# FatimaSohailll/KLT-Feature-Tracker-Acceleration-GPUs

Measured on AMD Instinct MI355X. Metric: frames/sec + pyramid Gpix/s @1080p 5000 feats, 1/2/4/8 MI355X, higher is better.
Workload: dtype f32; 1 GPU; 1920x1080, 5000 features, sequential KLTTrackFeatures pass + KLTStoreFeatureList per frame, 2361 frames per GPU (BASELINE config 3; config 5 at N>1); device-resident: frames in HBM before timing, features and table stay on the device (the API-inclusive figure is the `api` key); chunk=64, chunk_requested=64, resolution=1920x1080, features=5000, frames=2361, parallelism=single GPU, reduction=exact

## Files before the change

klt-feature-tracker-acceleration-gpus_amd/csrc/track7.hip:

```cpp
#pragma clang fp contract(off)
#pragma clang diagnostic ignored "-Wpass-failed"

#include <math.h>
#include <string.h>

#include "klt_dev.h"

#ifndef KLT_T7_PRED_UNIT
#define KLT_T7_PRED_UNIT 0
#endif
#ifndef KLT_T7_NL2
#define KLT_T7_NL2 1
#endif
#ifndef KLT_T7_REUSE
#define KLT_T7_REUSE 1
#endif
#ifndef KLT_T7_BATCH
#define KLT_T7_BATCH 7
#endif

namespace kltdev {
namespace {

constexpr int kWin = 7, kHw = 3, kNpx = kWin * kWin;
constexpr int kRow = 52;
constexpr int kRows = 6;
constexpr int kWaves = kBlock / kWave;

__device__ __forceinline__ float u(float v) { return __int_as_float(__builtin_amdgcn_readfirstlane(__float_as_int(v))); }
__device__ __forceinline__ int u(int v) { return __builtin_amdgcn_readfirstlane(v); }

#include "track7_solve.h"

constexpr int kThreeBits = 0x40400000;

__device__ __forceinline__ bool out7(float x, float y, int tx, int ty) {
  const int xb = __float_as_int(x), yb = __float_as_int(y);
  return xb < kThreeBits || xb >= tx || yb < kThreeBits || yb >= ty;
}

struct Pix {
  unsigned off;
  unsigned px;
  float w0, w1, w2, w3;
};

__device__ __forceinline__ Pix pix_at(int w, int h, float x, float y) {
  const int xt = (int)x, yt = (int)y;
  const float ax = x - xt, ay = y - yt;
  Pix p;
  p.px = (unsigned)(yt * w + xt);
  p.off = p.px * 4u;
  p.w0 = (1.0f - ax) * (1.0f - ay);
  p.w1 = ax * (1.0f - ay);
  p.w2 = (1.0f - ax) * ay;
  p.w3 = ax * ay;
  return p;
}

struct Quad {
  float2 r0, r1;
};

__device__ __forceinline__ Quad quad(const float *P, const Pix &p, unsigned rowb) {
  const char *b = reinterpret_cast<const char *>(P);
  const unsigned o1 = p.off + rowb;
  Quad q;
  q.r0 = *reinterpret_cast<const float2 *>(b + p.off);
  q.r1 = *reinterpret_cast<const float2 *>(b + o1);
  return q;
}

typedef float f4u __attribute__((ext_vector_type(4), aligned(4)));
typedef float f2u __attribute__((ext_vector_type(2), aligned(4)));
struct Tri {
  Quad i, x, y;
};
__device__ __forceinline__ Tri tri(const float *P, const Pix &p, unsigned rowb) {
  const char *base = reinterpret_cast<const char *>(P);
  const unsigned o0 = p.px * 12u, o1 = o0 + rowb;
  const f4u a0 = *reinterpret_cast<const f4u *>(base + o0), b0 = *reinterpret_cast<const f4u *>(base + o1);
  const f2u a1 = *reinterpret_cast<const f2u *>(base + o0 + 16), b1 = *reinterpret_cast<const f2u *>(base + o1 + 16);
  static_assert(kRecGx == 0 && kRecGy == 1 && kRecImg == 2, "record layout");
  Tri t;
  t.i.r0 = make_float2(a0.z, a1.y);
  t.i.r1 = make_float2(b0.z, b1.y);
  t.x.r0 = make_float2(a0.x, a0.w);
  t.x.r1 = make_float2(b0.x, b0.w);
  t.y.r0 = make_float2(a0.y, a1.x);
  t.y.r1 = make_float2(b0.y, b1.x);
  return t;
}
__device__ __forceinline__ Quad quad_i(const float *P, const Pix &p, unsigned rowb) {
  const unsigned o0 = p.px * 12u, o1 = o0 + rowb;
  const float *b = reinterpret_cast<const float *>(reinterpret_cast<const char *>(P) + o0);
  const float *c = reinterpret_cast<const float *>(reinterpret_cast<const char *>(P) + o1);
  Quad q;
  q.r0 = make_float2(b[kRecImg], b[kRec + kRecImg]);
  q.r1 = make_float2(c[kRecImg], c[kRec + kRecImg]);
  return q;
}

__device__ __forceinline__ float interp(const Pix &p, const Quad &q) {
  return p.w0 * q.r0.x + p.w1 * q.r0.y + p.w2 * q.r1.x + p.w3 * q.r1.y;
}

#ifndef KLT_T7_WAVEFENCE
#define KLT_T7_WAVEFENCE 1
#endif
__device__ __forceinline__ void wave_lds_sync() {
#if KLT_T7_WAVEFENCE
  __builtin_amdgcn_fence(__ATOMIC_RELEASE, "wavefront");
  __builtin_amdgcn_wave_barrier();
  __builtin_amdgcn_fence(__ATOMIC_ACQUIRE, "wavefront");
#else
  __builtin_amdgcn_fence(__ATOMIC_RELEASE, "workgroup");
  __builtin_amdgcn_wave_barrier();
  __builtin_amdgcn_fence(__ATOMIC_ACQUIRE, "workgroup");
#endif
}

typedef float f4 __attribute__((ext_vector_type(4)));

template <int NS, bool PIN = false>
__device__ __forceinline__ float sums7_acc(float *red, int lane, bool on, const float (&v)[NS]) {
  if (on) {
#pragma unroll
    for (int s = 0; s < NS; ++s) red[s * kRow + lane] = v[s];
  }
  wave_lds_sync();
  float acc = 0.0f;
  if constexpr (PIN) asm volatile("" : "+v"(lane));
  if (lane < NS) {
    const float *r = red + lane * kRow;
    constexpr int NCH = kRow / 4, B = KLT_T7_BATCH;
#pragma unroll
    for (int k0 = 0; k0 < NCH; k0 += B) {
      f4 c[B];
#pragma unroll
      for (int k = 0; k < B; ++k)
        if (k0 + k < NCH) c[k] = *reinterpret_cast<const f4 *>(r + 4 * (k0 + k));
#pragma unroll
      for (int k = 0; k < B; ++k) {
        const int q = 4 * (k0 + k);
        if (k0 + k >= NCH) break;
        acc += c[k].x;
        if (q + 1 < kNpx) acc += c[k].y;
        if (q + 2 < kNpx) acc += c[k].z;
        if (q + 3 < kNpx) acc += c[k].w;
      }
    }
  }
  wave_lds_sync();
  return acc;
}
template <int NS, bool PIN = false>
__device__ __forceinline__ void sums7(float *red, int lane, bool on, const float (&v)[NS], float (&out)[NS]) {
  const float acc = sums7_acc<NS, PIN>(red, lane, on, v);
#pragma unroll
  for (int s = 0; s < NS; ++s) out[s] = __int_as_float(__builtin_amdgcn_readlane(__float_as_int(acc), s));
}

constexpr int kQuadXor1 = 0xB1, kQuadXor2 = 0x4E, kRowRor4 = 0x124, kRowRor8 = 0x128;
constexpr int kRowBcast15 = 0x142, kRowBcast31 = 0x143;
#ifndef KLT_T7_BCAST
#define KLT_T7_BCAST 1
#endif
template <int CTRL>
__device__ __forceinline__ float dpp_add(float x) {
  return x + __int_as_float(__builtin_amdgcn_update_dpp(0, __float_as_int(x), CTRL, 0xF, 0xF, false));
}

template <int NS>
__device__ __forceinline__ void tree7(bool on, const float (&v)[NS], float (&out)[NS]) {
  float x[NS];
#pragma unroll
  for (int s = 0; s < NS; ++s) x[s] = on ? v[s] : 0.0f;
#pragma unroll
  for (int s = 0; s < NS; ++s) x[s] = dpp_add<kQuadXor1>(x[s]);
#pragma unroll
  for (int s = 0; s < NS; ++s) x[s] = dpp_add<kQuadXor2>(x[s]);
#pragma unroll
  for (int s = 0; s < NS; ++s) x[s] = dpp_add<kRowRor4>(x[s]);
#pragma unroll
  for (int s = 0; s < NS; ++s) x[s] = dpp_add<kRowRor8>(x[s]);
#if KLT_T7_BCAST
#pragma unroll
  for (int s = 0; s < NS; ++s) x[s] = x[s] + __int_as_float(__builtin_amdgcn_update_dpp(0, __float_as_int(x[s]),
                                                                                          kRowBcast15, 0xF, 0xF, true));
#pragma unroll
  for (int s = 0; s < NS; ++s) x[s] = x[s] + __int_as_float(__builtin_amdgcn_update_dpp(0, __float_as_int(x[s]),
                                                                                          kRowBcast31, 0xF, 0xF, true));
#pragma unroll
  for (int s = 0; s < NS; ++s) out[s] = __int_as_float(__builtin_amdgcn_readlane(__float_as_int(x[s]), 63));
#else
#pragma unroll
  for (int s = 0; s < NS; ++s) {
    const int b = __float_as_int(x[s]);
    out[s] = (__int_as_float(__builtin_amdgcn_readlane(b, 0)) + __int_as_float(__builtin_amdgcn_readlane(b, 16))) +
             (__int_as_float(__builtin_amdgcn_readlane(b, 32)) + __int_as_float(__builtin_amdgcn_readlane(b, 48)));
  }
#endif
}

template <int NS, bool FAST, bool PIN = false>
__device__ __forceinline__ void sums(float *red, int lane, bool on, const float (&v)[NS], float (&out)[NS]) {
  if constexpr (FAST) tree7<NS>(on, v, out);
  else sums7<NS, PIN>(red, lane, on, v, out);
}

constexpr int kPS = 24;
constexpr int kPatS = 16 * kPS, kPatT = 2 * 16 * 8, kPatG = 2 * 8 * 8;
constexpr int kPat = kPatS + kPatT;
static_assert(kPatG <= kPatS, "G over S");
constexpr int kRedF = kRows * kRow + 4;

typedef float f2 __attribute__((ext_vector_type(2)));

__device__ __forceinline__ void patch_load(const float *img, int w, int h, int X0, int Y0, int lane, float (&v)[4]) {
  const int sc = lane & 15, sr = 2 * ((lane >> 4) & 1) + (lane >> 5);
  const unsigned xc = (unsigned)clampi(X0 - kHw + sc, 0, w - 1);
  const char *b = reinterpret_cast<const char *>(img);
#pragma unroll
  for (int k = 0; k < 4; ++k) {
    const unsigned yc = (unsigned)clampi(Y0 - kHw + sr + 4 * k, 0, h - 1);
    v[k] = *reinterpret_cast<const float *>(b + (yc * (unsigned)w + xc) * 4u);
  }
}

__device__ __forceinline__ void patch_grads(float *pat, int lane, const TrkArgs &a, int w, int h, const float (&v)[4],
                                            int X0, int Y0, int cx, int cy, Quad &qi, Quad &qx, Quad &qy) {
  const int sc = lane & 15, sr = 2 * ((lane >> 4) & 1) + (lane >> 5);
#pragma unroll
  for (int k = 0; k < 4; ++k) pat[(sr + 4 * k) * kPS + sc] = v[k];
  wave_lds_sync();
  {
    const float *S = pat + (cy + kHw) * kPS + cx + kHw;
    qi.r0 = make_float2(S[0], S[1]);
    qi.r1 = make_float2(S[kPS], S[kPS + 1]);
  }
  const int c = lane & 7, r = lane >> 3;
#pragma unroll
  for (int k = 0; k < 2; ++k) {
    const float *row = pat + (r + 8 * k) * kPS + c;
    f2 t = {0.0f, 0.0f};
#pragma unroll
    for (int m = 0; m < 7; ++m) t += f2{row[m], row[m]} * f2{a.gd[m], a.gg[m]};
    float *T = pat + kPatS + 2 * ((r + 8 * k) * 8 + c);
    T[0] = t.y;
    T[1] = t.x;
  }
  wave_lds_sync();
  {
    const float *col = pat + kPatS + 2 * (r * 8 + c);
    f2 g = {0.0f, 0.0f};
#pragma unroll
    for (int m = 0; m < 7; ++m) g += *reinterpret_cast<const f2 *>(col + 16 * m) * f2{a.gd[m], a.gg[m]};
    const int x = X0 + c, y = Y0 + r;
    if (x < kHw || x + kHw >= w || y < kHw || y + kHw >= h) g = f2{0.0f, 0.0f};
    *reinterpret_cast<f2 *>(pat + 2 * (r * 8 + c)) = g;
  }
  wave_lds_sync();
  const int cx1 = min(cx + 1, 7), cy1 = min(cy + 1, 7);
  const f2 g00 = *reinterpret_cast<const f2 *>(pat + 2 * (cy * 8 + cx));
  const f2 g01 = *reinterpret_cast<const f2 *>(pat + 2 * (cy * 8 + cx1));
  const f2 g10 = *reinterpret_cast<const f2 *>(pat + 2 * (cy1 * 8 + cx));
  const f2 g11 = *reinterpret_cast<const f2 *>(pat + 2 * (cy1 * 8 + cx1));
  qx.r0 = make_float2(g00.y, g01.y);
  qx.r1 = make_float2(g10.y, g11.y);
  qy.r0 = make_float2(g00.x, g01.x);
  qy.r1 = make_float2(g10.x, g11.x);
  wave_lds_sync();
}

struct Carry {
  unsigned px = ~0u;
  Quad i, x, y;
};
#ifndef KLT_T7_CARRY
#define KLT_T7_CARRY 1
#endif

struct Lev {
  const float *img, *gx, *gy;
  int w, h, vlo, vhi;
  int tx, ty;
  int il;
};

__device__ __forceinline__ Lev lev_of(const TrkLevel &L, long off, int tx, int ty) {
  return Lev{L.img + off, L.gx + off, L.gy + off, L.w, L.h, L.vlo, L.vhi, tx, ty, L.il};
}

__device__ __forceinline__ Lev lev_prev(const TrkArgs &a, const TrkFramesArgs &b, int r, int j) {
  const TrkLevel &P = a.A[r], &Q = a.B[r];
  const bool f = j == 0;
  const long off = f ? 0L : (long)(j - 1) * b.lfs[r];
  return Lev{(f ? P.img : Q.img) + off, (f ? P.gx : Q.gx) + off, (f ? P.gy : Q.gy) + off, f ? P.w : Q.w,
             f ? P.h : Q.h, f ? P.vlo : Q.vlo, f ? P.vhi : Q.vhi, a.oobx[r], a.ooby[r], f ? P.il : Q.il};
}

template <bool MULTI>
__device__ __forceinline__ Lev lev_cur(const TrkArgs &a, const TrkFramesArgs &b, int r, int j, int sq, int nsq) {
  if constexpr (MULTI) return lev_of(a.B[r], ((long)j * nsq + sq) * b.lfs[r], a.oobx[r], a.ooby[r]);
  else return lev_of(a.B[r], (long)j * b.lfs[r], a.oobx[r], a.ooby[r]);
}
template <bool MULTI>
__device__ __forceinline__ Lev lev_before(const TrkArgs &a, const TrkFramesArgs &b, int r, int j, int sq, int nsq) {
  if constexpr (MULTI) {
    const TrkLevel &P = a.A[r], &Q = a.B[r];
    const bool f = j == 0;
    const long off = (f ? (long)sq : (long)(j - 1) * nsq + sq) * b.lfs[r];
    return Lev{(f ? P.img : Q.img) + off, nullptr, nullptr, Q.w, Q.h, Q.vlo, Q.vhi, a.oobx[r], a.ooby[r], Q.il};
  } else {
    return lev_prev(a, b, r, j);
  }
}

template <bool MULTI, bool ROLL>
__device__ __forceinline__ Lev lev_img1(const TrkArgs &a, const TrkFramesArgs &b, int r, int j, int sq, int nsq,
                                        const float *pimg, int pil) {
  if constexpr (ROLL) {
    const TrkLevel &Q = a.B[r];
    return Lev{pimg, nullptr, nullptr, Q.w, Q.h, Q.vlo, Q.vhi, a.oobx[r], a.ooby[r], pil};
  } else {
    return lev_before<MULTI>(a, b, r, j, sq, nsq);
  }
}

__device__ __forceinline__ bool band_bad(const Lev &L, float y) {
  return (int)(y - kHw) < L.vlo || (int)(y + kHw) + 1 >= L.vhi;
}

struct Pending {
  bool on = false;
  float x2 = 0.0f, y2 = 0.0f;
  int it = 0;
  float aim = 0.0f;
};

struct Counts {
  unsigned solves = 0, passes = 0;
#ifdef KLT_TRACK_PROF
  unsigned long long c[kProfN] = {};
#endif
};

constexpr int kWaveXcdShift = 60;
constexpr unsigned long long kWaveTimeMask = (1ull << kWaveXcdShift) - 1ull;
__device__ __forceinline__ void wave_time(unsigned long long *wave_t, int which, unsigned k) {
  const unsigned long long t = wall_clock64(), cap = wave_t[2];
  const unsigned long long xcd = (unsigned)__builtin_amdgcn_s_getreg((31 << 11) | 20) & 15u;
  if (k < cap) wave_t[4 + which * cap + k] = (t & kWaveTimeMask) | (xcd << kWaveXcdShift);
}
struct T7KArgs {
  TrkArgs a;
  TrkFramesArgs b;
  float *fx, *fy;
  int *fv;
  int n;
};
typedef const __attribute__((address_space(4))) T7KArgs *T7KArgsPtr;
__device__ __forceinline__ T7KArgsPtr t7_kargs() {
  return (T7KArgsPtr)__builtin_amdgcn_kernarg_segment_ptr();
}
__device__ __forceinline__ void wave_exit(int lane, unsigned k) {
  if (lane != 0) return;
  const T7KArgsPtr ka = t7_kargs();
  unsigned long long *const wave_t = ka->b.wave_t;
  unsigned *const exits = ka->b.exits;
  if (wave_t) wave_time(wave_t, 1, k);
  if (exits) {
    const unsigned k = atomicAdd(exits, 1u) + 1u;
    if (k == ka->b.exit_thr) __hip_atomic_store(ka->b.exit_sig, k, __ATOMIC_RELAXED, __HIP_MEMORY_SCOPE_SYSTEM);
  }
}

#ifdef KLT_TRACK_PROF
#define T7_T(t) const unsigned long long t = clock64()
#define T7_ADD(k, t0) cnt.c[k] += clock64() - (t0)
#else
#define T7_T(t)
#define T7_ADD(k, t0)
#endif

struct LevState {
  float x2, y2;
  float pxy;
  float aim, agx, agy;
  int it = 0;
  int status = kTracked;
  unsigned bpx = ~0u;
  Quad bi, bx, by;
};

enum { kPassAgain = 0, kPassDone = 1, kPassOOB = 2, kPassLostPrev = 3 };

template <bool BAND, bool FIRST, bool JOB, bool AOS, bool FAST, int LZ = 0>
__device__ __forceinline__ int pass7(const TrkArgs &a, const Lev &A, const Lev &B, float x1, float y1, bool x1_out,
                                     LevState &ls, int lane, float fi, float fj, bool on, float *red, Pending &pd,
                                     const Lev &R, int &rstat, Counts &cnt, const Carry &cr = Carry{},
                                     unsigned cpx = ~0u) {
  T7_T(t_top);
  if constexpr (KLT_T7_SOLVE2 && !FIRST) ls.x2 = lane_of(ls.pxy, 0), ls.y2 = lane_of(ls.pxy, 1);
  bool stop = (FIRST && x1_out) || out7(ls.x2, ls.y2, A.tx, A.ty);
  if (BAND && !stop && (band_bad(B, ls.y2) || (FIRST && band_bad(A, y1)))) {
    *a.escape = 1;
    stop = true;
  }
  if (stop) {
    ls.status = kOOB;
    if (JOB) {
      const Pix q = pix_at(R.w, R.h, pd.x2 + fi, pd.y2 + fj);
      const float rb =
          interp(q, AOS && !LZ ? quad_i(R.img, q, (unsigned)R.w * 12u) : quad(R.img, q, (unsigned)R.w * 4u));
      float v[1] = {on ? fabsf(pd.aim - rb) : 0.0f}, S[1];
      ++cnt.passes;
      sums<1, FAST, LZ != 0>(red, lane, on, v, S);
      rstat = S[0] / (float)kNpx > a.max_res ? kLargeResidue : (pd.it >= a.max_it ? kMaxIter : kTracked);
      pd.on = false;
      if (rstat != kTracked) return kPassLostPrev;
    }
    return kPassOOB;
  }
  T7_ADD(11, t_top);
  T7_T(t_g0);
  ++cnt.passes;
  const unsigned rowB = (unsigned)B.w * (AOS ? 12u : 4u);
  const Pix qb = pix_at(B.w, B.h, ls.x2 + fi, ls.y2 + fj);
  Quad bi, bx, by;
  const bool reuse = !FIRST && KLT_T7_REUSE && __ballot(qb.px != ls.bpx) == 0ull;
  Pix qa = qb, qr = qb;
  Quad ai{}, ax{}, ay{}, ri{};
  if constexpr (LZ == 2) {
    float *pat = red + kRedF;
    if (FIRST) qa = pix_at(A.w, A.h, x1 + fi, y1 + fj);
    if (JOB) {
      qr = pix_at(R.w, R.h, pd.x2 + fi, pd.y2 + fj);
      ri = quad(R.img, qr, (unsigned)R.w * 4u);
    }
    const int X0b = u((int)(ls.x2 - (float)kHw)), Y0b = u((int)(ls.y2 - (float)kHw));
    const int cxb = (int)(ls.x2 + fi) - X0b, cyb = (int)(ls.y2 + fj) - Y0b;
    const bool carry = FIRST && KLT_T7_CARRY && __ballot(qa.px != cpx) == 0ull;
    if (reuse) {
      bi = ls.bi;
      bx = ls.bx;
      by = ls.by;
    } else if (!FIRST || carry) {
      float v[4];
      patch_load(B.img, B.w, B.h, X0b, Y0b, lane, v);
      patch_grads(pat, lane, a, B.w, B.h, v, X0b, Y0b, cxb, cyb, bi, bx, by);
      if (FIRST) ai = cr.i, ax = cr.x, ay = cr.y;
    } else if (A.il == kLayoutImg) {
      const int X0a = u((int)(x1 - (float)kHw)), Y0a = u((int)(y1 - (float)kHw));
      float v[4], va[4];
      patch_load(B.img, B.w, B.h, X0b, Y0b, lane, v);
      patch_load(A.img, A.w, A.h, X0a, Y0a, lane, va);
      patch_grads(pat, lane, a, B.w, B.h, v, X0b, Y0b, cxb, cyb, bi, bx, by);
      patch_grads(pat, lane, a, A.w, A.h, va, X0a, Y0a, (int)(x1 + fi) - X0a, (int)(y1 + fj) - Y0a, ai, ax, ay);
    } else {
      float v[4];
      patch_load(B.img, B.w, B.h, X0b, Y0b, lane, v);
      const Tri t = tri(A.img, qa, (unsigned)A.w * 12u);
      patch_grads(pat, lane, a, B.w, B.h, v, X0b, Y0b, cxb, cyb, bi, bx, by);
      ai = t.i, ax = t.x, ay = t.y;
    }
  } else if (reuse) {
    bi = ls.bi;
    bx = ls.bx;
    by = ls.by;
  } else if constexpr (AOS) {
    const Tri t = tri(B.img, qb, rowB);
    bi = t.i;
    bx = t.x;
    by = t.y;
  } else {
    bi = quad(B.img, qb, rowB);
    bx = quad(B.gx, qb, rowB);
    by = quad(B.gy, qb, rowB);
  }
  if (KLT_T7_REUSE) {
    ls.bpx = qb.px;
    ls.bi = bi;
    ls.bx = bx;
    ls.by = by;
  }
  if (FIRST && LZ != 2) {
    const unsigned rowA = (unsigned)A.w * (AOS ? 12u : 4u);
    qa = pix_at(A.w, A.h, x1 + fi, y1 + fj);
    if constexpr (AOS) {
      const Tri t = tri(A.img, qa, rowA);
      ai = t.i;
      ax = t.x;
      ay = t.y;
    } else {
      ai = quad(A.img, qa, rowA);
      ax = quad(A.gx, qa, rowA);
      ay = quad(A.gy, qa, rowA);
    }
  }
  if (JOB && LZ != 2) {
    qr = pix_at(R.w, R.h, pd.x2 + fi, pd.y2 + fj);
    ri = AOS && !LZ ? quad_i(R.img, qr, (unsigned)R.w * 12u) : quad(R.img, qr, (unsigned)R.w * 4u);
  }
  if (FIRST) {
    ls.aim = interp(qa, ai);
    ls.agx = interp(qa, ax);
    ls.agy = interp(qa, ay);
  }
  const float bim = interp(qb, bi), bgx = interp(qb, bx), bgy = interp(qb, by);
  const float dif = ls.aim - bim, gxs = ls.agx + bgx, gys = ls.agy + bgy;
#ifdef KLT_TRACK_PROF
  asm volatile("" ::"v"(dif), "v"(gxs), "v"(gys));
#endif
  T7_ADD(0, t_g0);
  T7_T(t_s0);
  constexpr bool S2L = KLT_T7_SOLVE2 && !FAST;
  constexpr int iXX = S2L ? kSumGxx : 0, iXY = S2L ? kSumGxy : 1, iYY = S2L ? kSumGyy : 2, iEX = S2L ? kSumEx : 3,
                iEY = S2L ? kSumEy : 4, iRes = S2L ? kSumRes : 5;
  float S[6], acc = 0.0f;
  if (JOB) {
    const float rb = interp(qr, ri);
    float v[6];
    v[iXX] = gxs * gxs, v[iXY] = gxs * gys, v[iYY] = gys * gys, v[iEX] = dif * gxs, v[iEY] = dif * gys;
    v[iRes] = fabsf(pd.aim - rb);
    if constexpr (S2L) {
      acc = sums7_acc<6, LZ != 0>(red, lane, on, v);
      S[5] = lane_of(acc, kSumRes);
    } else {
      sums<6, FAST, LZ != 0>(red, lane, on, v, S);
    }
    rstat = S[5] / (float)kNpx > a.max_res ? kLargeResidue : (pd.it >= a.max_it ? kMaxIter : kTracked);
    pd.on = false;
    if (rstat != kTracked) return kPassLostPrev;
  } else {
    float v[5];
    v[iXX] = gxs * gxs, v[iXY] = gxs * gys, v[iYY] = gys * gys, v[iEX] = dif * gxs, v[iEY] = dif * gys;
    if constexpr (S2L) {
      acc = sums7_acc<5, LZ != 0>(red, lane, on, v);
    } else {
      float S5[5];
      sums<5, FAST, LZ != 0>(red, lane, on, v, S5);
#pragma unroll
      for (int k = 0; k < 5; ++k) S[k] = S5[k];
    }
  }
  T7_ADD(1, t_s0);
  T7_T(t_v0);
  ++cnt.solves;
  if constexpr (S2L) S[0] = lane_of(acc, kSumGxx), S[1] = lane_of(acc, kSumGxy), S[2] = lane_of(acc, kSumGyy);
  const float det = solve_det(S[0], S[1], S[2]);
  if (det < a.min_det) {
    ls.status = kSmallDet;
    return kPassDone;
  }
  bool moved;
  if constexpr (KLT_T7_SOLVE2) {
    float d;
    if constexpr (S2L) {
      d = solve2(acc, S[1], a.step, det);
    } else {
      int l = lane;
      if constexpr (LZ != 0) asm volatile("" : "+v"(l));
      const float S5[5] = {S[0], S[1], S[2], S[3], S[4]};
      d = solve2u(S5, l == 0, a.step, det);
    }
    ls.pxy += d;
    moved = (__ballot(fabsf(d) >= a.min_disp) & 3ull) != 0ull;
  } else {
    const float S5[5] = {S[0], S[1], S[2], S[3], S[4]};
    float dx, dy;
    solve1(S5, a.step, det, dx, dy);
    dx = u(dx);
    dy = u(dy);
    ls.x2 = u(ls.x2 + dx);
    ls.y2 = u(ls.y2 + dy);
    moved = fabsf(dx) >= a.min_disp || fabsf(dy) >= a.min_disp;
  }
  ++ls.it;
  T7_ADD(2, t_v0);
  return (moved && ls.it < a.max_it) ? kPassAgain : kPassDone;
}

template <bool BAND, bool AOS, bool FAST, int LZ = 0>
__device__ int level7(const TrkArgs &a, const Lev &A, const Lev &B, float x1, float y1, float &x2, float &y2,
                      int lane, float fi, float fj, bool on, float *red, bool residue, bool defer, Pending &pd,
                      bool job, const Lev &R, int &rstat, bool &lost_prev, Counts &cnt, Carry *cr = nullptr,
                      unsigned cpx = ~0u) {
  const bool x1_out = out7(x1, y1, A.tx, A.ty);
  LevState ls;
  ls.x2 = x2;
  ls.y2 = y2;
  ls.pxy = x2;
  asm("s_nop 1\n\tv_writelane_b32 %0, %1, 1" : "+v"(ls.pxy) : "s"(y2));
  const Carry none{};
  const Carry &c0 = LZ == 2 ? *cr : none;
  int r = job ? pass7<BAND, true, true, AOS, FAST, LZ>(a, A, B, x1, y1, x1_out, ls, lane, fi, fj, on, red, pd, R, rstat,
                                                       cnt, c0, cpx)
              : pass7<BAND, true, false, AOS, FAST, LZ>(a, A, B, x1, y1, x1_out, ls, lane, fi, fj, on, red, pd, R, rstat,
                                                        cnt, c0, cpx);
  while (r == kPassAgain)
    r = pass7<BAND, false, false, AOS, FAST, LZ>(a, A, B, x1, y1, x1_out, ls, lane, fi, fj, on, red, pd, R, rstat, cnt);
  if constexpr (KLT_T7_SOLVE2) ls.x2 = lane_of(ls.pxy, 0), ls.y2 = lane_of(ls.pxy, 1);
  x2 = ls.x2;
  y2 = ls.y2;
  if constexpr (LZ == 2 && KLT_T7_CARRY && KLT_T7_REUSE) {
    cr->px = ls.bpx;
    cr->i = ls.bi;
    cr->x = ls.bx;
    cr->y = ls.by;
  }
  if (r == kPassLostPrev) {
    lost_prev = true;
    return kTracked;
  }
  if (r == kPassOOB) return kOOB;
  if (out7(x2, y2, A.tx, A.ty)) return kOOB;
  if (BAND && band_bad(B, y2)) {
    *a.escape = 1;
    return kOOB;
  }
  if (ls.status == kSmallDet) return kSmallDet;
  if (!residue) return ls.it >= a.max_it ? kMaxIter : kTracked;
  if (defer) {
    pd.on = true;
    pd.x2 = x2;
    pd.y2 = y2;
    pd.it = ls.it;
    pd.aim = ls.aim;
    return kTracked;
  }
  ++cnt.passes;
  T7_T(t_r0);
  const Pix q = pix_at(B.w, B.h, x2 + fi, y2 + fj);
  const float rb =
      interp(q, AOS && LZ != 2 ? quad_i(B.img, q, (unsigned)B.w * 12u) : quad(B.img, q, (unsigned)B.w * 4u));
  float v[1] = {on ? fabsf(ls.aim - rb) : 0.0f}, S1[1];
  sums<1, FAST, LZ != 0>(red, lane, on, v, S1);
  T7_ADD(3, t_r0);
  if (S1[0] / (float)kNpx > a.max_res) return kLargeResidue;
  return ls.it >= a.max_it ? kMaxIter : kTracked;
}

template <bool BAND, bool AOS, int NL, bool FAST = false, bool LAZY = false>
__global__ __launch_bounds__(kBlock, LAZY && NL == 2 ? 5 : LAZY ? 4 : 1) void k_track7(TrkArgs a, TrkFramesArgs b, float *__restrict__ fx,
                                                   float *__restrict__ fy, int *__restrict__ fv, int n) {
  static_assert(!LAZY || (AOS && !BAND), "lazy gradients: whole-frame interleaved pyramids");
  __shared__ __attribute__((aligned(16))) float red_all[kWaves][kRedF + (LAZY ? kPat : 0)];
  constexpr bool FB = false, HOOK = false, MULTI = false, PRED = false;
  const TrkFbArgs fb{};
  const TrkMultiArgs ms{};
  const TrkPredArgs pr{};
#include "track7_body.h"
}

template <int NL, bool FAST>
__global__ __launch_bounds__(kBlock, NL == 2 ? 5 : 4) void k_track7_hook(TrkArgs a, TrkFramesArgs b,
                                                                          float *__restrict__ fx,
                                                                          float *__restrict__ fy,
                                                                          int *__restrict__ fv, int n) {
  __shared__ __attribute__((aligned(16))) float red_all[kWaves][kRedF + kPat];
  constexpr bool BAND = false, AOS = true, LAZY = true, FB = false, HOOK = true, MULTI = false, PRED = false;
  const TrkFbArgs fb{};
  const TrkMultiArgs ms{};
  const TrkPredArgs pr{};
#include "track7_body.h"
}

template <bool AOS, int NL>
__global__ __launch_bounds__(kBlock) void k_track7_fb(TrkArgs a, TrkFramesArgs b, TrkFbArgs fb,
                                                      float *__restrict__ fx, float *__restrict__ fy,
                                                      int *__restrict__ fv, int n) {
  __shared__ __attribute__((aligned(16))) float red_all[kWaves][kRedF];
  constexpr bool BAND = false, FAST = false, FB = true, LAZY = false, HOOK = false, MULTI = false, PRED = false;
  const TrkMultiArgs ms{};
  const TrkPredArgs pr{};
#include "track7_body.h"
}

template <int NL>
__global__ __launch_bounds__(kBlock) void k_track7_multi(TrkArgs a, TrkFramesArgs b, TrkMultiArgs ms,
                                                         float *__restrict__ fx, float *__restrict__ fy,
                                                         int *__restrict__ fv, int n) {
  __shared__ __attribute__((aligned(16))) float red_all[kWaves][kRedF];
  constexpr bool BAND = false, AOS = true, FAST = false, FB = false, LAZY = false, HOOK = false, MULTI = true,
                 PRED = false;
  const TrkFbArgs fb{};
  const TrkPredArgs pr{};
#include "track7_body.h"
}

template <bool AOS, int NL>
__global__ __launch_bounds__(kBlock) void k_track7_pred(TrkArgs a, TrkFramesArgs b, TrkPredArgs pr,
                                                        float *__restrict__ fx, float *__restrict__ fy,
                                                        int *__restrict__ fv, int n) {
  __shared__ __attribute__((aligned(16))) float red_all[kWaves][kRedF];
  constexpr bool BAND = false, FAST = false, FB = false, LAZY = false, HOOK = false, MULTI = false, PRED = true;
  const TrkFbArgs fb{};
  const TrkMultiArgs ms{};
#include "track7_body.h"
}

}

static int oob_threshold(int n) {
  auto out = [n](int xb) {
    float x;
    memcpy(&x, &xb, sizeof x);
    volatile float t = x + 3.0f;
    volatile float g = (float)n - t;
    return g < 1.001f;
  };
  const float c = (float)(n > 3 ? n : 3);
  int lo, hi;
  const float three = 3.0f;
  memcpy(&lo, &three, sizeof lo);
  memcpy(&hi, &c, sizeof hi);
  if (out(lo)) return lo;
  while (hi - lo > 1) {
    const int mid = lo + (hi - lo) / 2;
    if (out(mid)) hi = mid;
    else lo = mid;
  }
  return hi;
}

#if KLT_T7_PRED_UNIT
hipError_t launch_track7_pred(hipStream_t st, const TrkArgs &a, const TrkFramesArgs &b, const TrkPredArgs &pr, float *x,
                              float *y, int *v, int n, int grid, bool two, const char **name) {
  if (name)
    *name = a.aos && two ? "kltdev::k_track7_pred<true, 2>"
            : a.aos      ? "kltdev::k_track7_pred<true, 0>"
                         : "kltdev::k_track7_pred<false, 0>";
  if (a.aos && two)
    hipLaunchKernelGGL((k_track7_pred<true, 2>), dim3(grid), dim3(kBlock), 0, st, a, b, pr, x, y, v, n);
  else if (a.aos)
    hipLaunchKernelGGL((k_track7_pred<true, 0>), dim3(grid), dim3(kBlock), 0, st, a, b, pr, x, y, v, n);
  else
    hipLaunchKernelGGL((k_track7_pred<false, 0>), dim3(grid), dim3(kBlock), 0, st, a, b, pr, x, y, v, n);
  return hipGetLastError();
}
#else
hipError_t launch_track7_multi(hipStream_t st, const TrkArgs &a_in, const TrkFramesArgs &b, const TrkMultiArgs &m,
                               float *x, float *y, int *v, int n, const char **name) {
  if (!a_in.aos || a_in.fast || a_in.lazy || a_in.escape || m.nseq < 1 || m.nseq > kMaxSeq || m.first[0] != 0 ||
      m.first[m.nseq] != n || b.perm || b.n_dev || b.xcd_per)
    return hipErrorInvalidValue;
  TrkArgs a = a_in;
  for (int l = 0; l < KLT_HIP_MAX_LEVELS; ++l) {
    a.oobx[l] = oob_threshold(a.B[l].w);
    a.ooby[l] = oob_threshold(a.B[l].h);
  }
  const int grid = (n + kWaves - 1) / kWaves;
  const bool two = KLT_T7_NL2 && a.nlev == 2;
  if (name) *name = two ? "kltdev::k_track7_multi<2>" : "kltdev::k_track7_multi<0>";
  if (two) hipLaunchKernelGGL((k_track7_multi<2>), dim3(grid), dim3(kBlock), 0, st, a, b, m, x, y, v, n);
  else hipLaunchKernelGGL((k_track7_multi<0>), dim3(grid), dim3(kBlock), 0, st, a, b, m, x, y, v, n);
  return hipGetLastError();
}

hipError_t launch_track7(hipStream_t st, bool band, const TrkArgs &a_in, const TrkFramesArgs &b, float *x, float *y,
                         int *v, int n, const char **name, const TrkFbArgs *fb, const TrkPredArgs *pr) {
  TrkArgs a = a_in;
  for (int l = 0; l < KLT_HIP_MAX_LEVELS; ++l) {
    a.oobx[l] = oob_threshold(a.B[l].w);
    a.ooby[l] = oob_threshold(a.B[l].h);
  }
  const int nb = (n + kWaves - 1) / kWaves;
  const int grid = b.xcd_per > 0 ? 8 * b.xcd_per : nb;
  const bool two = KLT_T7_NL2 && a.nlev == 2;
  if (fb) {
    if (band || a.fast || pr) return hipErrorInvalidValue;
    if (name)
      *name = a.aos && two ? "kltdev::k_track7_fb<true, 2>"
              : a.aos      ? "kltdev::k_track7_fb<true, 0>"
                           : "kltdev::k_track7_fb<false, 0>";
    if (a.aos && two)
      hipLaunchKernelGGL((k_track7_fb<true, 2>), dim3(grid), dim3(kBlock), 0, st, a, b, *fb, x, y, v, n);
    else if (a.aos)
      hipLaunchKernelGGL((k_track7_fb<true, 0>), dim3(grid), dim3(kBlock), 0, st, a, b, *fb, x, y, v, n);
    else
      hipLaunchKernelGGL((k_track7_fb<false, 0>), dim3(grid), dim3(kBlock), 0, st, a, b, *fb, x, y, v, n);
    return hipGetLastError();
  }
  if (pr) {
    if (band || a.fast || a.lazy || !pr->vx || !pr->vy) return hipErrorInvalidValue;
    return launch_track7_pred(st, a, b, *pr, x, y, v, n, grid, two, name);
  }
  if (a.lazy) {
    if (band || !a.aos || (a.fast && !two)) return hipErrorInvalidValue;
    if (a.B[0].il != kLayoutImg) return hipErrorInvalidValue;
    for (int l = 0; l < a.nlev; ++l)
      if (a.A[l].w != a.B[l].w || a.A[l].h != a.B[l].h) return hipErrorInvalidValue;
    if (name)
      *name = a.fast ? "kltdev::k_track7<false, true, 2, true, true>"
              : two  ? "kltdev::k_track7<false, true, 2, false, true>"
                     : "kltdev::k_track7<false, true, 0, false, true>";
    if (b.exits || b.wave_t) {
      if (name)
        *name = a.fast ? "kltdev::k_track7_hook<2, true>"
                : two  ? "kltdev::k_track7_hook<2, false>"
                       : "kltdev::k_track7_hook<0, false>";
      if (a.fast)
        hipLaunchKernelGGL((k_track7_hook<2, true>), dim3(grid), dim3(kBlock), 0, st, a, b, x, y, v, n);
      else if (two)
        hipLaunchKernelGGL((k_track7_hook<2, false>), dim3(grid), dim3(kBlock), 0, st, a, b, x, y, v, n);
      else
        hipLaunchKernelGGL((k_track7_hook<0, false>), dim3(grid), dim3(kBlock), 0, st, a, b, x, y, v, n);
      return hipGetLastError();
    }
    if (a.fast)
      hipLaunchKernelGGL((k_track7<false, true, 2, true, true>), dim3(grid), dim3(kBlock), 0, st, a, b, x, y, v, n);
    else if (two)
      hipLaunchKernelGGL((k_track7<false, true, 2, false, true>), dim3(grid), dim3(kBlock), 0, st, a, b, x, y, v, n);
    else
      hipLaunchKernelGGL((k_track7<false, true, 0, false, true>), dim3(grid), dim3(kBlock), 0, st, a, b, x, y, v, n);
    return hipGetLastError();
  }
  if (name)
    *name = a.fast ? (band ? "kltdev::k_track7<true, true, 2, true>" : "kltdev::k_track7<false, true, 2, true>")
            : band && a.aos && two ? "kltdev::k_track7<true, true, 2, false>"
            : a.aos && two         ? "kltdev::k_track7<false, true, 2, false>"
            : band && a.aos        ? "kltdev::k_track7<true, true, 0, false>"
            : band                 ? "kltdev::k_track7<true, false, 0, false>"
            : a.aos                ? "kltdev::k_track7<false, true, 0, false>"
                                   : "kltdev::k_track7<false, false, 0, false>";
  if (a.fast) {
    if (band)
      hipLaunchKernelGGL((k_track7<true, true, 2, true>), dim3(grid), dim3(kBlock), 0, st, a, b, x, y, v, n);
    else
      hipLaunchKernelGGL((k_track7<false, true, 2, true>), dim3(grid), dim3(kBlock), 0, st, a, b, x, y, v, n);
  } else if (band && a.aos && two)
    hipLaunchKernelGGL((k_track7<true, true, 2>), dim3(grid), dim3(kBlock), 0, st, a, b, x, y, v, n);
  else if (a.aos && two)
    hipLaunchKernelGGL((k_track7<false, true, 2>), dim3(grid), dim3(kBlock), 0, st, a, b, x, y, v, n);
  else if (band && a.aos)
    hipLaunchKernelGGL((k_track7<true, true, 0>), dim3(grid), dim3(kBlock), 0, st, a, b, x, y, v, n);
  else if (band)
    hipLaunchKernelGGL((k_track7<true, false, 0>), dim3(grid), dim3(kBlock), 0, st, a, b, x, y, v, n);
  else if (a.aos)
    hipLaunchKernelGGL((k_track7<false, true, 0>), dim3(grid), dim3(kBlock), 0, st, a, b, x, y, v, n);
  else
    hipLaunchKernelGGL((k_track7<false, false, 0>), dim3(grid), dim3(kBlock), 0, st, a, b, x, y, v, n);
  return hipGetLastError();
}
#endif

}
```

klt-feature-tracker-acceleration-gpus_amd/csrc/track7_body.h:

```cpp
  constexpr bool LATE = LAZY && !FB && !MULTI;
  static_assert(!PRED || (!FB && !MULTI && !LAZY && !BAND && !FAST && !HOOK), "k_track7_pred: full records, exact sums");
  static_assert(!HOOK || LATE, "wave_exit reads T7KArgs");
  if (a.prio) __builtin_amdgcn_s_setprio(3);
  const int lane = threadIdx.x & (kWave - 1), wave = threadIdx.x / kWave;
  if constexpr (HOOK)
    if (b.wave_t && lane == 0) wave_time(b.wave_t, 0, blockIdx.x * kWaves + wave);
  if (b.n_dev) n = *b.n_dev;
  const int xcd_per = b.n_dev && b.xcd_per > 0 ? ((n + kWaves - 1) / kWaves + 7) / 8 : b.xcd_per;
  if (xcd_per > 0 && (int)(blockIdx.x / 8) >= xcd_per) {
    if constexpr (HOOK) wave_exit(lane, blockIdx.x * kWaves + wave);
    return;
  }
  const int blk = xcd_per > 0 ? (int)(blockIdx.x % 8) * xcd_per + (int)(blockIdx.x / 8) : (int)blockIdx.x;
  const int slot = blk * kWaves + wave;
  if (slot >= n) {
    if constexpr (HOOK) wave_exit(lane, slot);
    return;
  }
  const int f = u(b.perm ? b.perm[slot] : slot);
  int sq = 0, nsq = 1;
  if constexpr (MULTI) {
    nsq = ms.nseq;
    int hi = nsq;
    while (hi - sq > 1) {
      const int mid = (sq + hi) >> 1;
      if (f >= ms.first[mid]) sq = mid;
      else hi = mid;
    }
    sq = u(sq);
  }
  float *red = red_all[wave];
  for (int i = lane; i < kRedF; i += kWave) red[i] = 0.0f;
  wave_lds_sync();
  const bool on = lane < kNpx;
  const int pl = on ? lane : kNpx - 1;
  const float fi = (float)(pl % kWin - kHw), fj = (float)(pl / kWin - kHw);

  float x = u(fx[f]), y = u(fy[f]);
  int v = u(fv[f]);
  const int nlev = NL > 0 ? NL : a.nlev;
  const bool merge = !FB && !PRED && a.merge_res && nlev >= 2;
  float pvx = 0.0f, pvy = 0.0f;
  if constexpr (PRED) pvx = u(pr.vx[f]), pvy = u(pr.vy[f]);
  Pending pd;
  Counts cnt;
  Carry carry;
#ifdef KLT_TRACK_PROF
  const unsigned long long wall0 = wall_clock64();
#endif
  constexpr bool ROLL = LAZY && NL > 0 && !FB && !MULTI;
  const float *pimg[NL > 0 ? NL : 1] = {};
  int pil = kLayoutImg;
  if constexpr (ROLL) {
#pragma unroll
    for (int r = 0; r < NL; ++r) pimg[r] = a.A[r].img;
    pil = a.A[0].il;
  }
  for (int j = 0; j < b.nframes; ++j) {
    T7_T(t_f0);
    const bool job = pd.on;
    const float xp = x, yp = y;
    int rstat = kTracked;
    if constexpr (PRED)
      if (v != 0) pvx = 0.0f, pvy = 0.0f;
    if (v >= 0 || job) {
      const Lev R = lev_img1<MULTI, ROLL>(a, b, 0, j, sq, nsq, pimg[0], pil);
      const unsigned cpx = carry.px;
      carry.px = ~0u;
      float xl = x, yl = y;
#pragma unroll
      for (int r = nlev - 1; r >= 0; --r) {
        xl = u(a.ss_inv != 0.0f ? xl * a.ss_inv : xl / a.ss);
        yl = u(a.ss_inv != 0.0f ? yl * a.ss_inv : yl / a.ss);
      }
      float xo = xl, yo = yl;
      if constexpr (PRED) {
        xo = u(x + pvx);
        yo = u(y + pvy);
#pragma unroll
        for (int r = nlev - 1; r >= 0; --r) {
          xo = u(a.ss_inv != 0.0f ? xo * a.ss_inv : xo / a.ss);
          yo = u(a.ss_inv != 0.0f ? yo * a.ss_inv : yo / a.ss);
        }
      }
      int val = kTracked;
      bool lost_prev = false;
#pragma unroll
      for (int r = nlev - 1; r >= 0; --r) {
        xl = u(xl * a.ss);
        yl = u(yl * a.ss);
        xo = u(xo * a.ss);
        yo = u(yo * a.ss);
        const Lev LA = lev_img1<MULTI, ROLL>(a, b, r, j, sq, nsq, pimg[ROLL ? r : 0], pil);
        const Lev LB = lev_cur<MULTI>(a, b, r, j, sq, nsq);
        if constexpr (PRED)
          if (r == nlev - 1) {
            const bool in = !out7(xo, yo, LB.tx, LB.ty);
            xo = u(in ? xo : xl);
            yo = u(in ? yo : yl);
          }
        const bool lj = job && r == nlev - 1;
        T7_T(t_l0);
        if (LAZY && r == 0)
          val = level7<BAND, AOS, FAST, LAZY ? 2 : 0>(a, LA, LB, xl, yl, xo, yo, lane, fi, fj, on, red, true,
                                                      merge && j + 1 < b.nframes, pd, lj, R, rstat, lost_prev, cnt,
                                                      &carry, cpx);
        else
          val = level7<BAND, AOS, FAST, LAZY ? 1 : 0>(a, LA, LB, xl, yl, xo, yo, lane, fi, fj, on, red, r == 0,
                           merge && r == 0 && j + 1 < b.nframes, pd, lj, R, rstat, lost_prev, cnt);
        T7_ADD(10, t_l0);
        if (lost_prev) break;
        if (val == kSmallDet || val == kOOB) break;
      }
      if (!lost_prev) {
        const bool border = xo < a.borderx || xo > a.ncols - 1 - a.borderx || yo < a.bordery ||
                            yo > a.nrows - 1 - a.bordery;
        if (val == kOOB || border) {
          pd.on = false;
          x = -1.0f;
          y = -1.0f;
          v = kOOB;
        } else if (val != kTracked) {
          x = -1.0f;
          y = -1.0f;
          v = val;
        } else {
          x = xo;
          y = yo;
          v = kTracked;
        }
      }
    }
    if constexpr (PRED) {
      pvx = v == kTracked ? u(x - xp) : 0.0f;
      pvy = v == kTracked ? u(y - yp) : 0.0f;
      if (pr.tvx && lane == 0) {
        pr.tvx[j * pr.tstride + f] = pvx;
        pr.tvy[j * pr.tstride + f] = pvy;
      }
    }
    if constexpr (FB) {
      float e = -1.0f;
      if (v == kTracked) {
        float xl = x, yl = y;
#pragma unroll
        for (int r = nlev - 1; r >= 0; --r) {
          xl = u(a.ss_inv != 0.0f ? xl * a.ss_inv : xl / a.ss);
          yl = u(a.ss_inv != 0.0f ? yl * a.ss_inv : yl / a.ss);
        }
        float xo = xl, yo = yl;
        int vb = kTracked;
        bool none = false;
        const Lev R = lev_prev(a, b, 0, j);
#pragma unroll
        for (int r = nlev - 1; r >= 0; --r) {
          xl = u(xl * a.ss);
          yl = u(yl * a.ss);
          xo = u(xo * a.ss);
          yo = u(yo * a.ss);
          const Lev LA = lev_of(a.B[r], (long)j * b.lfs[r], a.oobx[r], a.ooby[r]);
          const Lev LB = lev_prev(a, b, r, j);
          vb = level7<false, AOS, false>(a, LA, LB, xl, yl, xo, yo, lane, fi, fj, on, red, r == 0, false, pd, false, R,
                                         rstat, none, cnt);
          if (vb == kSmallDet || vb == kOOB) break;
        }
        const bool border = xo < a.borderx || xo > a.ncols - 1 - a.borderx || yo < a.bordery ||
                            yo > a.nrows - 1 - a.bordery;
        bool rej = vb != kTracked || border;
        if (!rej) {
          const float dx = xo - xp, dy = yo - yp;
          const float dx2 = dx * dx, dy2 = dy * dy;
          e = u(dx2 + dy2);
          rej = e > fb.t2;
        }
        if (rej) {
          x = -1.0f;
          y = -1.0f;
          v = kFbRejected;
        }
      }
      if (fb.err && lane == 0) fb.err[j * fb.stride + f] = e;
    }
    int tl = lane;
    if constexpr (LATE) asm volatile("" : "+v"(tl));
    if (job) {
      if (rstat != kTracked) {
        x = -1.0f;
        y = -1.0f;
        v = rstat;
      }
      if (b.tx && tl == 0) {
        b.tx[(j - 1) * b.tstride + f] = rstat != kTracked ? -1.0f : xp;
        b.ty[(j - 1) * b.tstride + f] = rstat != kTracked ? -1.0f : yp;
        b.tv[(j - 1) * b.tstride + f] = rstat;
      }
    }
    if (b.tx && tl == 0 && !pd.on) {
      b.tx[j * b.tstride + f] = x;
      b.ty[j * b.tstride + f] = y;
      b.tv[j * b.tstride + f] = v;
    }
    if constexpr (ROLL) {
#pragma unroll
      for (int r = 0; r < NL; ++r) pimg[r] = a.B[r].img + (long)j * b.lfs[r];
      pil = kLayoutImg;
    }
    T7_ADD(4, t_f0);
  }
#ifdef KLT_TRACK_PROF
  cnt.c[5] = cnt.solves;
  cnt.c[6] = cnt.passes;
  cnt.c[8] = wall0;
  cnt.c[9] = wall_clock64();
  cnt.c[7] = cnt.c[9] - wall0;
  if (b.prof && lane == 0)
    for (int k = 0; k < kProfN; ++k) b.prof[(long)slot * kProfN + k] = cnt.c[k];
#endif
  if (lane == 0) {
    float *ox = fx, *oy = fy;
    int *ov = fv;
    unsigned long long *count = nullptr;
    if constexpr (LATE) {
      const T7KArgsPtr ka = t7_kargs();
      ox = ka->fx, oy = ka->fy, ov = ka->fv, count = ka->b.count;
    } else {
      count = b.count;
    }
    ox[f] = x;
    oy[f] = y;
    ov[f] = v;
    if constexpr (PRED) {
      pr.vx[f] = pvx;
      pr.vy[f] = pvy;
    }
    if (count) {
      const int k = slot & (kCountSlots - 1);
      atomicAdd(&count[k], (unsigned long long)cnt.solves);
      atomicAdd(&count[kCountSlots + k], (unsigned long long)cnt.passes);
    }
  }
  if constexpr (HOOK) wave_exit(lane, f);
```

Measured before the change: 129,200 frames/s.

## Move deferred residue verdict onto level-0 first pass, reusing the level-0 interpolated patch

```diff
diff --git a/klt-feature-tracker-acceleration-gpus_amd/csrc/track7.hip b/klt-feature-tracker-acceleration-gpus_amd/csrc/track7.hip
--- a/klt-feature-tracker-acceleration-gpus_amd/csrc/track7.hip
+++ b/klt-feature-tracker-acceleration-gpus_amd/csrc/track7.hip
@@ -14,6 +14,9 @@
 #endif
 #ifndef KLT_T7_REUSE
 #define KLT_T7_REUSE 1
+#endif
+#ifndef KLT_T7_RES0
+#define KLT_T7_RES0 1
 #endif
 #ifndef KLT_T7_BATCH
 #define KLT_T7_BATCH 7
@@ -384,6 +387,16 @@
 #define T7_ADD(k, t0)
 #endif
 
+template <bool FAST>
+__device__ __forceinline__ int verdict7(const TrkArgs &a, const Lev &R, float x, float y, float aim, int ok, int lane,
+                                        float fi, float fj, bool on, float *red) {
+  const Pix q = pix_at(R.w, R.h, x + fi, y + fj);
+  const float rb = interp(q, quad(R.img, q, (unsigned)R.w * 4u));
+  float v[1] = {on ? fabsf(aim - rb) : 0.0f}, S[1];
+  sums<1, FAST, true>(red, lane, on, v, S);
+  return S[0] / (float)kNpx > a.max_res ? kLargeResidue : ok;
+}
+
 struct LevState {
   float x2, y2;
   float pxy;
@@ -396,7 +409,7 @@
 
 enum { kPassAgain = 0, kPassDone = 1, kPassOOB = 2, kPassLostPrev = 3 };
 
-template <bool BAND, bool FIRST, bool JOB, bool AOS, bool FAST, int LZ = 0>
+template <bool BAND, bool FIRST, bool JOB, bool AOS, bool FAST, int LZ = 0, bool R0 = false>
 __device__ __forceinline__ int pass7(const TrkArgs &a, const Lev &A, const Lev &B, float x1, float y1, bool x1_out,
                                      LevState &ls, int lane, float fi, float fj, bool on, float *red, Pending &pd,
                                      const Lev &R, int &rstat, Counts &cnt, const Carry &cr = Carry{},
@@ -410,7 +423,7 @@
   }
   if (stop) {
     ls.status = kOOB;
-    if (JOB) {
+    if (JOB && !R0) {
       const Pix q = pix_at(R.w, R.h, pd.x2 + fi, pd.y2 + fj);
       const float rb =
           interp(q, AOS && !LZ ? quad_i(R.img, q, (unsigned)R.w * 12u) : quad(R.img, q, (unsigned)R.w * 4u));
@@ -435,7 +448,7 @@
   if constexpr (LZ == 2) {
     float *pat = red + kRedF;
     if (FIRST) qa = pix_at(A.w, A.h, x1 + fi, y1 + fj);
-    if (JOB) {
+    if (JOB && !R0) {
       qr = pix_at(R.w, R.h, pd.x2 + fi, pd.y2 + fj);
       ri = quad(R.img, qr, (unsigned)R.w * 4u);
     }
@@ -520,7 +533,10 @@
                 iEY = S2L ? kSumEy : 4, iRes = S2L ? kSumRes : 5;
   float S[6], acc = 0.0f;
   if (JOB) {
-    const float rb = interp(qr, ri);
+    static_assert(!R0 || LZ == 2, "R0: the job rides level 0's first pass");
+    float rb;
+    if constexpr (R0) rb = ls.aim;
+    else rb = interp(qr, ri);
     float v[6];
     v[iXX] = gxs * gxs, v[iXY] = gxs * gys, v[iYY] = gys * gys, v[iEX] = dif * gxs, v[iEY] = dif * gys;
     v[iRes] = fabsf(pd.aim - rb);
@@ -530,9 +546,16 @@
     } else {
       sums<6, FAST, LZ != 0>(red, lane, on, v, S);
     }
-    rstat = S[5] / (float)kNpx > a.max_res ? kLargeResidue : (pd.it >= a.max_it ? kMaxIter : kTracked);
-    pd.on = false;
-    if (rstat != kTracked) return kPassLostPrev;
+    if constexpr (R0) {
+      if (rstat > 0) {
+        rstat = S[5] / (float)kNpx > a.max_res ? kLargeResidue : 1 - rstat;
+        if (rstat != kTracked) return kPassLostPrev;
+      }
+    } else {
+      rstat = S[5] / (float)kNpx > a.max_res ? kLargeResidue : (pd.it >= a.max_it ? kMaxIter : kTracked);
+      pd.on = false;
+      if (rstat != kTracked) return kPassLostPrev;
+    }
   } else {
     float v[5];
     v[iXX] = gxs * gxs, v[iXY] = gxs * gys, v[iYY] = gys * gys, v[iEX] = dif * gxs, v[iEY] = dif * gys;
@@ -582,11 +605,11 @@
   return (moved && ls.it < a.max_it) ? kPassAgain : kPassDone;
 }
 
-template <bool BAND, bool AOS, bool FAST, int LZ = 0>
+template <bool BAND, bool AOS, bool FAST, int LZ = 0, bool R0 = false>
 __device__ int level7(const TrkArgs &a, const Lev &A, const Lev &B, float x1, float y1, float &x2, float &y2,
                       int lane, float fi, float fj, bool on, float *red, bool residue, bool defer, Pending &pd,
                       bool job, const Lev &R, int &rstat, bool &lost_prev, Counts &cnt, Carry *cr = nullptr,
-                      unsigned cpx = ~0u) {
+                      unsigned cpx = ~0u, int *its = nullptr) {
   const bool x1_out = out7(x1, y1, A.tx, A.ty);
   LevState ls;
   ls.x2 = x2;
@@ -595,12 +618,21 @@
   asm("s_nop 1\n\tv_writelane_b32 %0, %1, 1" : "+v"(ls.pxy) : "s"(y2));
   const Carry none{};
   const Carry &c0 = LZ == 2 ? *cr : none;
-  int r = job ? pass7<BAND, true, true, AOS, FAST, LZ>(a, A, B, x1, y1, x1_out, ls, lane, fi, fj, on, red, pd, R, rstat,
-                                                       cnt, c0, cpx)
-              : pass7<BAND, true, false, AOS, FAST, LZ>(a, A, B, x1, y1, x1_out, ls, lane, fi, fj, on, red, pd, R, rstat,
-                                                        cnt, c0, cpx);
+  int r;
+  if constexpr (R0 && LZ != 2)
+    r = pass7<BAND, true, false, AOS, FAST, LZ>(a, A, B, x1, y1, x1_out, ls, lane, fi, fj, on, red, pd, R, rstat, cnt,
+                                                c0, cpx);
+  else if constexpr (R0)
+    r = pass7<BAND, true, true, AOS, FAST, LZ, true>(a, A, B, x1, y1, x1_out, ls, lane, fi, fj, on, red, pd, R, rstat,
+                                                     cnt, c0, cpx);
+  else
+    r = job ? pass7<BAND, true, true, AOS, FAST, LZ>(a, A, B, x1, y1, x1_out, ls, lane, fi, fj, on, red, pd, R, rstat,
+                                                     cnt, c0, cpx)
+            : pass7<BAND, true, false, AOS, FAST, LZ>(a, A, B, x1, y1, x1_out, ls, lane, fi, fj, on, red, pd, R, rstat,
+                                                      cnt, c0, cpx);
   while (r == kPassAgain)
     r = pass7<BAND, false, false, AOS, FAST, LZ>(a, A, B, x1, y1, x1_out, ls, lane, fi, fj, on, red, pd, R, rstat, cnt);
+  if constexpr (R0 && LZ != 2) *its = ls.it;
   if constexpr (KLT_T7_SOLVE2) ls.x2 = lane_of(ls.pxy, 0), ls.y2 = lane_of(ls.pxy, 1);
   x2 = ls.x2;
   y2 = ls.y2;
@@ -790,6 +822,9 @@
   if (a.lazy) {
     if (band || !a.aos || (a.fast && !two)) return hipErrorInvalidValue;
     if (a.B[0].il != kLayoutImg) return hipErrorInvalidValue;
+#if KLT_T7_RES0
+    if (a.ss_inv == 0.0f) a.merge_res = 0;
+#endif
     for (int l = 0; l < a.nlev; ++l)
       if (a.A[l].w != a.B[l].w || a.A[l].h != a.B[l].h) return hipErrorInvalidValue;
     if (name)
diff --git a/klt-feature-tracker-acceleration-gpus_amd/csrc/track7_body.h b/klt-feature-tracker-acceleration-gpus_amd/csrc/track7_body.h
--- a/klt-feature-tracker-acceleration-gpus_amd/csrc/track7_body.h
+++ b/klt-feature-tracker-acceleration-gpus_amd/csrc/track7_body.h
@@ -49,6 +49,8 @@
   const unsigned long long wall0 = wall_clock64();
 #endif
   constexpr bool ROLL = LAZY && NL > 0 && !FB && !MULTI;
+  constexpr bool RES0 = KLT_T7_RES0 && LAZY && NL == 2 && !FB && !MULTI && !PRED;
+  constexpr int kVerdictNone = -64;
   const float *pimg[NL > 0 ? NL : 1] = {};
   int pil = kLayoutImg;
   if constexpr (ROLL) {
@@ -61,6 +63,10 @@
     const bool job = pd.on;
     const float xp = x, yp = y;
     int rstat = kTracked;
+    if constexpr (RES0) {
+      rstat = !job ? kVerdictNone : 1 - (pd.it >= a.max_it ? kMaxIter : kTracked);
+      pd.on = false;
+    }
     if constexpr (PRED)
       if (v != 0) pvx = 0.0f, pvy = 0.0f;
     if (v >= 0 || job) {
@@ -85,6 +91,7 @@
       }
       int val = kTracked;
       bool lost_prev = false;
+      unsigned k1 = 0;
 #pragma unroll
       for (int r = nlev - 1; r >= 0; --r) {
         xl = u(xl * a.ss);
@@ -99,18 +106,35 @@
             xo = u(in ? xo : xl);
             yo = u(in ? yo : yl);
           }
-        const bool lj = job && r == nlev - 1;
+        const bool lj = job && r == (RES0 ? 0 : nlev - 1);
         T7_T(t_l0);
         if (LAZY && r == 0)
-          val = level7<BAND, AOS, FAST, LAZY ? 2 : 0>(a, LA, LB, xl, yl, xo, yo, lane, fi, fj, on, red, true,
-                                                      merge && j + 1 < b.nframes, pd, lj, R, rstat, lost_prev, cnt,
-                                                      &carry, cpx);
-        else
+          val = level7<BAND, AOS, FAST, LAZY ? 2 : 0, RES0>(a, LA, LB, xl, yl, xo, yo, lane, fi, fj, on, red, true,
+                                                            merge && j + 1 < b.nframes, pd, lj, R, rstat, lost_prev,
+                                                            cnt, &carry, cpx);
+        else if constexpr (RES0) {
+          int it1 = 0;
+          val = level7<BAND, AOS, FAST, 1, true>(a, LA, LB, xl, yl, xo, yo, lane, fi, fj, on, red, false, false, pd,
+                                                 false, R, rstat, lost_prev, cnt, nullptr, ~0u, &it1);
+          k1 = (unsigned)it1 + (val == kSmallDet ? 1u : 0u);
+        } else
           val = level7<BAND, AOS, FAST, LAZY ? 1 : 0>(a, LA, LB, xl, yl, xo, yo, lane, fi, fj, on, red, r == 0,
                            merge && r == 0 && j + 1 < b.nframes, pd, lj, R, rstat, lost_prev, cnt);
         T7_ADD(10, t_l0);
         if (lost_prev) break;
         if (val == kSmallDet || val == kOOB) break;
+      }
+      if constexpr (RES0) {
+        if (rstat > 0) {
+          rstat = verdict7<FAST>(a, R, xp, yp, pd.aim, 1 - rstat, lane, fi, fj, on, red);
+          lost_prev = rstat != kTracked;
+          if (k1 == 0 || lost_prev) ++cnt.passes;
+        }
+        if (lost_prev) {
+          cnt.solves -= k1;
+          cnt.passes -= k1;
+          carry.px = ~0u;
+        }
       }
       if (!lost_prev) {
         const bool border = xo < a.borderx || xo > a.ncols - 1 - a.borderx || yo < a.bordery ||
@@ -183,7 +207,9 @@
     }
     int tl = lane;
     if constexpr (LATE) asm volatile("" : "+v"(tl));
-    if (job) {
+    bool judged = job;
+    if constexpr (RES0) judged = (unsigned)-rstat < (unsigned)-kVerdictNone;
+    if (judged) {
       if (rstat != kTracked) {
         x = -1.0f;
         y = -1.0f;
```

Result: no change. 128,300 frames/s (-0.7%).
